# TencentARC/Mix-of-Show

Measured on AMD Instinct MI355X. Metric: edlora_train_images_per_sec_512_sd15, higher is better.
Workload: dtype fp16; 1 GPU; BASELINE.json configs[1]: single-concept ED-LoRA tune, SD-1.5 UNet/CLIP/VAE (random init, calibrated), 512x512, LoRA rank 4 on Attention+CLIPAttention, attn_reg on, batch 4/GPU; global_batch=4, per_gpu_batch=4, image_size=512, parallelism=dp1, grad_bucket_bytes=4466688, preset=sd15, hipgraph=True, channels_last=True

## Files before the change

include/mos_hip.h:

```cpp
#ifndef MOS_HIP_H
#define MOS_HIP_H

#include <stdint.h>

#ifdef __cplusplus
extern "C" {
#endif

typedef enum { MOS_F16 = 0, MOS_BF16 = 1 } mos_dtype;

typedef enum {
    MOS_OK = 0,
    MOS_ERR_BAD_ARG = -1,
    MOS_ERR_UNSUPPORTED = -2,
    MOS_ERR_LAUNCH = -3
} mos_status;

#define MOS_LORA_PAD 16
#define MOS_MAX_PCOLS 4
#define MOS_MAX_SOURCES 9

int mos_version(void);
const char* mos_last_error_string(void);

// ... 75 lines not shown
    mos_lora_grad_out out;
} mos_lora_final_rec;
int mos_lora_linear_fused_bwd_deferred(const void* dy, int64_t lddy, const void* x, int64_t ldx,
                                       const void* Wt, int64_t ldwt, const void* t,
                                       const void* A16T, const void* BpT,
                                       void* dt, void* dx, int64_t lddx,
                                       const mos_lora_grad_out* grads_host, void* ws,
                                       int M, int N, int K, int lora_cols, int dtype, void* stream,
                                       mos_lora_final_rec* rec_host);
int mos_lora_grad_final_all(const mos_lora_final_rec* recs_dev, int n_recs, int total_blocks, void* stream);

typedef struct {
    const void* P[2];
    const void* Z[2];
    int64_t ldz[2];
    int C[2], cb[2];
    float* partial[2];
    int M, rpc, nchunk, nj;
    int block_begin, n_blocks;
    double flops, bytes;
} mos_lora_grad_job;
int mos_lora_linear_fused_bwd_deferred_all(const void* dy, int64_t lddy, const void* x, int64_t ldx,
                                           const void* Wt, int64_t ldwt, const void* t,
                                           const void* A16T, const void* BpT,
                                           void* dt, void* dx, int64_t lddx,
                                           const mos_lora_grad_out* grads_host, void* ws,
                                           int M, int N, int K, int lora_cols, int dtype, void* stream,
                                           mos_lora_final_rec* rec_host, mos_lora_grad_job* job_host);
int mos_lora_grad_all(const mos_lora_grad_job* jobs_dev, int n_jobs, int total_blocks, int nj, int dtype, double flops, double bytes,
                      void* stream);

typedef struct {
    int B, H, Nq, Nkv, d;
    int64_t q_bs, q_rs;
    int64_t k_bs, k_rs;
    int64_t v_bs, v_rs;
    int64_t o_bs, o_rs;
    float scale;
    int causal;
} mos_attn_shape;

int mos_attn_fwd(const void* q, const void* k, const void* v, void* o, float* lse,
                 const int32_t* tok_idx, int n_pcols, float* pcols,
                 const mos_attn_shape* shape_host, int dtype, void* stream);

typedef struct {
    int64_t do_bs, do_rs;
    int64_t dq_bs, dq_rs;
    int64_t dk_bs, dk_rs;
    int64_t dv_bs, dv_rs;
} mos_attn_grad_strides;

int64_t mos_attn_bwd_workspace_bytes(const mos_attn_shape* shape_host);
int mos_attn_bwd(const void* q, const void* k, const void* v, const void* o, const float* lse,
                 const void* dO, const int32_t* tok_idx, int n_pcols, const float* pcols,
                 const float* dpcols, void* dq, void* dk, void* dv, void* ws,
                 const mos_attn_shape* shape_host, const mos_attn_grad_strides* gs_host,
                 int dtype, void* stream);

int mos_self_attn_fwd(const void* q, const void* k, const void* v, void* o, float* lse,
                      const mos_attn_shape* shape_host, int dtype, void* stream);
int mos_cross_attn_fwd(const void* q, const void* k, const void* v, void* o, float* lse,
                       const int32_t* tok_idx, int n_pcols, float* pcols,
                       const mos_attn_shape* shape_host, int dtype, void* stream);
int mos_self_attn_bwd(const void* q, const void* k, const void* v, const void* o, const float* lse, const void* dO,
                      void* dq, void* dk, void* dv, void* ws, const mos_attn_shape* shape_host,
                      const mos_attn_grad_strides* gs_host, int dtype, void* stream);
int mos_cross_attn_bwd(const void* q, const void* k, const void* v, const void* o, const float* lse, const void* dO,
                       const int32_t* tok_idx, int n_pcols, const float* pcols, const float* dpcols,
                       void* dq, void* dk, void* dv, void* ws, const mos_attn_shape* shape_host,
                       const mos_attn_grad_strides* gs_host, int dtype, void* stream);

typedef struct {
    int n_regions;
    int feat_h, feat_w;
    int box[MOS_MAX_SOURCES - 1][4];
    int64_t src_stride;
} mos_region_desc;

int mos_region_cross_attn_fwd(const void* q, const void* k_src, const void* v_src, void* o,
                              const mos_attn_shape* shape_host, const mos_region_desc* reg_host,
                              int dtype, void* stream);
int mos_region_cross_attn_fwd_chunk(const void* q, const void* k_src, const void* v_src, void* o,
                                    const mos_attn_shape* shape_host, const mos_region_desc* reg_host,
                                    const void* total_count, int accumulate, int dtype, void* stream);

int mos_attn_probs(const void* q, const void* k, void* probs, const mos_attn_shape* shape_host, int dtype, void* stream);
int mos_attn_pv(const void* probs, const void* v, void* o, const mos_attn_shape* shape_host, int dtype, void* stream);
int64_t mos_attn_probs_bwd_workspace_bytes(const mos_attn_shape* shape_host);
int mos_attn_pv_bwd(const void* probs, const void* v, const void* dO, void* dprobs, void* dv, void* ws,
                    const mos_attn_shape* shape_host, const mos_attn_grad_strides* gs_host, int dtype, void* stream);
int mos_attn_probs_bwd(const void* q, const void* k, const void* probs, const void* dprobs, void* dq, void* dk, void* ws,
                       const mos_attn_shape* shape_host, const mos_attn_grad_strides* gs_host, int dtype, void* stream);

int64_t mos_gram_workspace_bytes(int64_t n, int Cin, int Cout);
int mos_gram_accumulate(const void* X, int64_t ldx, const void* Y, int64_t ldy, int64_t n,
                        int Cin, int Cout, int dtype, double* G, double* P, double* c,
                        void* ws, void* stream);
int64_t mos_lsq_workspace_bytes(int Cout, int Cin);

int mos_lsq_loss_grad_gram(const double* W, const double* G, const double* P, const double* c,
                           double n_times_cout, int Cout, int Cin, double* loss, double* grad,
                           void* ws, void* stream);

int64_t mos_groupnorm_workspace_bytes(int B, int C, int HW, int G);
int mos_groupnorm_silu_fwd(const void* x, const float* gamma, const float* beta, void* y, float* stats,
// ... 59 lines not shown
```

mix-of-show_amd/csrc/mos_attn.hip:

```cpp
#include <cstdio>
#include <cstdlib>
#include <type_traits>
#include "mos_common.h"

#ifndef MOS_DQ_OCC
#define MOS_DQ_OCC 2
#endif
#ifndef MOS_ATTN_PV16
#define MOS_ATTN_PV16 1
#endif

namespace {

constexpr float LOG2E = 1.4426950408889634f;
constexpr float NEG_BIG = -1.0e30f;
constexpr int KV_TILE = 64;
constexpr int TS = KV_TILE + 8;
__device__ __forceinline__ constexpr int tr_col(int c) { return (c & ~12) | ((c & 4) << 1) | ((c & 8) >> 1); }

__device__ __forceinline__ constexpr int tr_col16(int c) {
    return (c & 32) | ((((c >> 2) & 1) * 2 + ((c >> 4) & 1)) << 3) | (((c >> 3) & 1) << 2) | (c & 3);
}

template <int D>
// ... 1337 lines not shown
        asm volatile("" : "+v"(dvT[0]), "+v"(dkT[0]), "+v"(dvT[1]), "+v"(dkT[1]), "+v"(s1), "+v"(dp1), "+v"(pf1[0]), "+v"(dsf1[0]), "+v"(fdo10[0]), "+v"(fq10[0]), "+v"(fdo10[1]), "+v"(fq10[1]));
        #pragma unroll
        for (int dt = 0; dt < DT; ++dt) { fdo11[dt] = tr_afrag<T>(dOt + (32 * dt + l31) * TS, 1, 1, hh); fq11[dt] = tr_afrag<T>(Qt + (32 * dt + l31) * TS, 1, 1, hh); }
        dvT[0] = MT<T>::mfma32(fdo10[0], pf1[0], dvT[0]);
        { const float p = __builtin_amdgcn_exp2f(s1[8] * c - l1[2][0]); s1[8] = p; dp1[8] = p * dp1[8]; }
        { const float p = __builtin_amdgcn_exp2f(s1[9] * c - l1[2][1]); s1[9] = p; dp1[9] = p * dp1[9]; }
        asm volatile("" : "+v"(dvT[0]), "+v"(dkT[0]), "+v"(dvT[1]), "+v"(dkT[1]), "+v"(s1), "+v"(dp1));
        dkT[0] = MT<T>::mfma32(fq10[0], dsf1[0], dkT[0]);
        { const float p = __builtin_amdgcn_exp2f(s1[10] * c - l1[2][2]); s1[10] = p; dp1[10] = p * dp1[10]; }
        { const float p = __builtin_amdgcn_exp2f(s1[11] * c - l1[2][3]); s1[11] = p; dp1[11] = p * dp1[11]; }
        asm volatile("" : "+v"(dvT[0]), "+v"(dkT[0]), "+v"(dvT[1]), "+v"(dkT[1]), "+v"(s1), "+v"(dp1));
        dvT[1] = MT<T>::mfma32(fdo10[1], pf1[0], dvT[1]);
        { const float p = __builtin_amdgcn_exp2f(s1[12] * c - l1[3][0]); s1[12] = p; dp1[12] = p * dp1[12]; }
        { const float p = __builtin_amdgcn_exp2f(s1[13] * c - l1[3][1]); s1[13] = p; dp1[13] = p * dp1[13]; }
        asm volatile("" : "+v"(dvT[0]), "+v"(dkT[0]), "+v"(dvT[1]), "+v"(dkT[1]), "+v"(s1), "+v"(dp1));
        dkT[1] = MT<T>::mfma32(fq10[1], dsf1[0], dkT[1]);
        { const float p = __builtin_amdgcn_exp2f(s1[14] * c - l1[3][2]); s1[14] = p; dp1[14] = p * dp1[14]; }
        { const float p = __builtin_amdgcn_exp2f(s1[15] * c - l1[3][3]); s1[15] = p; dp1[15] = p * dp1[15]; }
        pf1[1] = acc_to_bfrag<T>(s1, 1); dsf1[1] = acc_to_bfrag<T>(dp1, 1);
        asm volatile("" : "+v"(dvT[0]), "+v"(dkT[0]), "+v"(dvT[1]), "+v"(dkT[1]), "+v"(s1), "+v"(dp1), "+v"(pf1[1]), "+v"(dsf1[1]), "+v"(fdo11[0]), "+v"(fq11[0]), "+v"(fdo11[1]), "+v"(fq11[1]));
        dvT[0] = MT<T>::mfma32(fdo11[0], pf1[1], dvT[0]);
        dkT[0] = MT<T>::mfma32(fq11[0], dsf1[1], dkT[0]);
        dvT[1] = MT<T>::mfma32(fdo11[1], pf1[1], dvT[1]);
        dkT[1] = MT<T>::mfma32(fq11[1], dsf1[1], dkT[1]);
        if (more) store_tile(cur ^ 1);
        __syncthreads();
        cur ^= 1;
    }
    if (a.nsplit == 1) {
        T* dkp = (T*)a.dk + (int64_t)b * a.dk_bs + (int64_t)kvi * a.dk_rs + h * D;
        T* dvp = (T*)a.dv + (int64_t)b * a.dv_bs + (int64_t)kvi * a.dv_rs + h * D;
        store_out_rows<T, D>(dkp, kvalid, dkT, a.scale, hh);
        store_out_rows<T, D>(dvp, kvalid, dvT, 1.0f, hh);
    } else if (kvalid) {
        const int64_t bh = (int64_t)b * a.H + h;
        const int64_t slab = (int64_t)a.B * a.H * a.Nkv * D;
        float* pk = a.part + ((int64_t)split * slab) + (bh * a.Nkv + kvi) * D;
        float* pv = pk + (int64_t)a.nsplit * slab;
#pragma unroll
        for (int dt = 0; dt < DT; ++dt)
#pragma unroll
            for (int r4 = 0; r4 < 4; ++r4) {
                const int db = 32 * dt + 8 * r4 + 4 * hh;
                if (db < D) {
                    *reinterpret_cast<f32x4*>(pk + db) = f32x4{dkT[dt][4 * r4] * a.scale, dkT[dt][4 * r4 + 1] * a.scale,
                                                              dkT[dt][4 * r4 + 2] * a.scale, dkT[dt][4 * r4 + 3] * a.scale};
                    *reinterpret_cast<f32x4*>(pv + db) = f32x4{dvT[dt][4 * r4], dvT[dt][4 * r4 + 1], dvT[dt][4 * r4 + 2],
                                                              dvT[dt][4 * r4 + 3]};
                }
            }
    }
}

template <int D> constexpr int fwd_qw() { return D <= 80 ? 64 : 32; }

template <int D> constexpr size_t fwd_lds(size_t es) { return 2 * (HD<D>::ROW_TILE_ELEMS + HD<D>::TR_TILE_ELEMS) * es; }
template <int D> constexpr size_t dq_lds(size_t es) { return 2 * (2 * HD<D>::ROW_TILE_ELEMS + HD<D>::TR_TILE_ELEMS) * es; }
template <int D> constexpr size_t dkdv_lds(size_t es) {
    return DKDV_NBUF<D>::value * ((2 * HD<D>::ROW_TILE_ELEMS + 2 * HD<D>::TR_TILE_ELEMS) * es +
                                  KV_TILE * (2 + MOS_MAX_PCOLS) * sizeof(float));
}

template <typename K>
void set_lds(K kernel, size_t bytes) {
    if (bytes > 48 * 1024)
        (void)hipFuncSetAttribute(reinterpret_cast<const void*>(kernel), hipFuncAttributeMaxDynamicSharedMemorySize, (int)bytes);
}

int check_shape(const mos_attn_shape* s, const char* who) {
    if (!s) return mos_set_error(MOS_ERR_BAD_ARG, "%s: NULL shape", who);
    if (s->B <= 0 || s->H <= 0 || s->Nq <= 0 || s->Nkv <= 0)
        return mos_set_error(MOS_ERR_BAD_ARG, "%s: B=%d H=%d Nq=%d Nkv=%d", who, s->B, s->H, s->Nq, s->Nkv);
    if (s->d != 40 && s->d != 64 && s->d != 80 && s->d != 160)
        return mos_set_error(MOS_ERR_UNSUPPORTED, "%s: head dim %d not in {40, 64, 80, 160}", who, s->d);
    if (s->causal && s->Nq != s->Nkv)
        return mos_set_error(MOS_ERR_BAD_ARG, "%s: causal masking needs Nq == Nkv (got %d, %d)", who, s->Nq, s->Nkv);
    if (s->q_rs % 8 || s->k_rs % 8 || s->v_rs % 8 || s->o_rs % 4 || s->q_bs % 8 || s->k_bs % 8 || s->v_bs % 8 || s->o_bs % 4)
        return mos_set_error(MOS_ERR_BAD_ARG, "%s: strides must be multiples of 8 elements", who);
    return MOS_OK;
}

AttnArgs make_args(const void* q, const void* k, const void* v, void* o, float* lse, const int32_t* tok, int np,
                   float* pcols, const mos_attn_shape* s, int q_tile) {
    AttnArgs a;
    a.q = q; a.k = k; a.v = v; a.o = o; a.lse = lse; a.tok_idx = tok; a.pcols = pcols; a.n_pcols = np;
    a.B = s->B; a.H = s->H; a.Nq = s->Nq; a.Nkv = s->Nkv; a.nqb = (s->Nq + q_tile - 1) / q_tile;
    a.q_bs = s->q_bs; a.q_rs = s->q_rs; a.k_bs = s->k_bs; a.k_rs = s->k_rs;
    a.v_bs = s->v_bs; a.v_rs = s->v_rs; a.o_bs = s->o_bs; a.o_rs = s->o_rs; a.scale = s->scale;
    a.causal = s->causal;
    return a;
}

template <typename T>
const char* tname() { return sizeof(T) == 2 && std::is_same<T, f16_t>::value ? "f16" : "bf16"; }

struct AttnKey {
    char s[96];
    double flops, bytes;
    AttnKey(const char* dt, const mos_attn_shape* sh, double gemms) {
        snprintf(s, sizeof(s), "%s d%d B%d H%d Nq%d Nkv%d", dt, sh->d, sh->B, sh->H, sh->Nq, sh->Nkv);
        flops = gemms * 2.0 * sh->B * sh->H * (double)sh->Nq * sh->Nkv * sh->d;
        bytes = 2.0 * sh->B * sh->H * sh->d * (2.0 * sh->Nq + 2.0 * sh->Nkv);
    }
};

template <int D> constexpr bool has_causal() { return true; }

template <typename T, int D, int QW, bool PCOLS, bool CAUSAL>
void launch_fwd_one(const AttnArgs& a, size_t lds, hipStream_t st) {
    const dim3 grid((unsigned)(a.H * a.nqb * a.B));
    set_lds(&attn_fwd_kernel<T, D, QW, PCOLS, CAUSAL>, lds);
    hipLaunchKernelGGL((attn_fwd_kernel<T, D, QW, PCOLS, CAUSAL>), grid, dim3(256), lds, st, a);
}
template <typename T, int D, int QW>
void launch_fwd_qw(const AttnArgs& a, int np, size_t lds, hipStream_t st) {
    if constexpr (has_causal<D>()) {
        if (a.causal) {
            if (np > 0) launch_fwd_one<T, D, QW, true, true>(a, lds, st);
            else launch_fwd_one<T, D, QW, false, true>(a, lds, st);
            return;
        }
    }
    if (np > 0) launch_fwd_one<T, D, QW, true, false>(a, lds, st);
    else launch_fwd_one<T, D, QW, false, false>(a, lds, st);
}

template <typename T, int D>
int launch_fwd(const void* q, const void* k, const void* v, void* o, float* lse, const int32_t* tok, int np,
               float* pcols, const mos_attn_shape* s, hipStream_t st) {
    constexpr int QW = fwd_qw<D>();
    const size_t lds = fwd_lds<D>(sizeof(T));
    AttnKey key(tname<T>(), s, 2.0);
    MosProfScope prof(st, np > 0 ? "attn_fwd_pcols" : "attn_fwd", key.s, key.flops, key.bytes);
    const int64_t wg_big = (int64_t)s->H * s->B * ((s->Nq + 4 * QW - 1) / (4 * QW));
    if (QW == 64 && wg_big < 512) {
        launch_fwd_qw<T, D, 32>(make_args(q, k, v, o, lse, tok, np, pcols, s, 128), np, lds, st);
    } else {
        launch_fwd_qw<T, D, QW>(make_args(q, k, v, o, lse, tok, np, pcols, s, 4 * QW), np, lds, st);
    }
    return mos_check_launch("attn_fwd");
}

template <typename T, int D>
int launch_region(const void* q, const void* k, const void* v, void* o, const mos_attn_shape* s,
                  const mos_region_desc* reg, const unsigned char* total_count, int accumulate, hipStream_t st) {
    AttnArgs a = make_args(q, k, v, o, nullptr, nullptr, 0, nullptr, s, 128);
    a.nqb = ((reg->feat_w + 15) / 16) * ((reg->feat_h + 7) / 8);
    const dim3 grid((unsigned)(a.H * a.nqb * a.B));
    const size_t lds = RG<D>::lds_bytes(sizeof(T));
    set_lds(&region_attn_kernel<T, D>, lds);
    double cover = 0.0, area = 0.0;
    for (int r = 0; r < reg->n_regions; ++r) {
        const double bh = reg->box[r][2] - reg->box[r][0], bw = reg->box[r][3] - reg->box[r][1];
        if (bh > 0 && bw > 0) area += bh * bw;
    }
    cover = area + (double)s->Nq;
    AttnKey key(tname<T>(), s, 2.0);
    char rk[128];
    snprintf(rk, sizeof(rk), "%s R%d", key.s, reg->n_regions);
    MosProfScope prof(st, "region_attn", rk, key.flops * cover / (double)s->Nq, key.bytes);
    hipLaunchKernelGGL((region_attn_kernel<T, D>), grid, dim3(256), lds, st, a, *reg, total_count, accumulate);
    return mos_check_launch("region_attn");
}

struct BwdPlan { int nw_q, nw_k, nqb, nkb, nsplit, q_per_split; };
BwdPlan plan_bwd(const mos_attn_shape* s) {
    BwdPlan p;
    p.nw_q = 4;
    p.nw_k = 4;
    p.nqb = (s->Nq + 32 * p.nw_q - 1) / (32 * p.nw_q);
    p.nkb = (s->Nkv + 32 * p.nw_k - 1) / (32 * p.nw_k);
    const int64_t base = (int64_t)p.nkb * s->B * s->H;
    const int qtiles = (s->Nq + KV_TILE - 1) / KV_TILE;
    int ns = (int)((512 + base - 1) / base);
    if (ns > qtiles) ns = qtiles;
    if (ns < 1) ns = 1;
    int tps = (qtiles + ns - 1) / ns;
    ns = (qtiles + tps - 1) / tps;
    p.nsplit = ns;
    p.q_per_split = tps * KV_TILE;
    return p;
}

template <typename T, int D>
int launch_bwd(const void* q, const void* k, const void* v, const void* o, const float* lse, const void* dO,
               const int32_t* tok, int np, const float* pcols, const float* dpcols, void* dq, void* dk, void* dv,
               void* ws, const mos_attn_shape* s, const mos_attn_grad_strides* g, hipStream_t st) {
    const BwdPlan p = plan_bwd(s);
    float* Dvec = (float*)ws;
    const int64_t nrows = (int64_t)s->B * s->H * s->Nq;
    float* part = Dvec + ((nrows + 3) / 4) * 4;
    AttnBwdArgs a;
    a.q = q; a.k = k; a.v = v; a.dO = dO; a.lse = lse; a.Dvec = Dvec; a.tok_idx = tok; a.dpcols = dpcols;
    a.o = o; a.o_bs = s->o_bs; a.o_rs = s->o_rs; a.pcols = pcols;
    a.n_pcols = (dpcols != nullptr && pcols != nullptr) ? np : 0;
    a.dq = dq; a.dk = dk; a.dv = dv; a.part = part;
    a.B = s->B; a.H = s->H; a.Nq = s->Nq; a.Nkv = s->Nkv; a.nqb = p.nqb; a.nkb = p.nkb;
    a.nsplit = p.nsplit; a.q_per_split = p.q_per_split;
    a.q_bs = s->q_bs; a.q_rs = s->q_rs; a.k_bs = s->k_bs; a.k_rs = s->k_rs; a.v_bs = s->v_bs; a.v_rs = s->v_rs;
    a.do_bs = g->do_bs; a.do_rs = g->do_rs; a.dq_bs = g->dq_bs; a.dq_rs = g->dq_rs;
    a.dk_bs = g->dk_bs; a.dk_rs = g->dk_rs; a.dv_bs = g->dv_bs; a.dv_rs = g->dv_rs; a.scale = s->scale;
    a.causal = s->causal;
    const bool pc = a.n_pcols > 0;
    {
        const dim3 grid((unsigned)(a.H * a.nqb * a.B));
        const size_t lds = dq_lds<D>(sizeof(T));
        AttnKey key(tname<T>(), s, 3.0);
        MosProfScope prof(st, "attn_bwd_dq", key.s, key.flops, key.bytes * 1.5);
        auto go = [&](auto pc_c, auto ca_c) {
            constexpr bool PC = decltype(pc_c)::value, CA = decltype(ca_c)::value;
            set_lds(&attn_bwd_dq_kernel<T, D, PC, 4, CA>, lds);
            hipLaunchKernelGGL((attn_bwd_dq_kernel<T, D, PC, 4, CA>), grid, dim3(256), lds, st, a);
        };
        bool done = false;
        if constexpr (has_causal<D>()) {
            if (a.causal) {
                if (pc) go(std::true_type{}, std::true_type{}); else go(std::false_type{}, std::true_type{});
                done = true;
            }
        }
        if (!done) { if (pc) go(std::true_type{}, std::false_type{}); else go(std::false_type{}, std::false_type{}); }
        int rc = mos_check_launch("attn_bwd_dq");
        if (rc) return rc;
    }
    {
        const dim3 grid((unsigned)(a.H * a.nkb * a.B), (unsigned)a.nsplit);
        const size_t lds = dkdv_lds<D>(sizeof(T));
        AttnKey key(tname<T>(), s, 4.0);
        MosProfScope prof(st, "attn_bwd_dkdv", key.s, key.flops, key.bytes * 1.5);
        auto go = [&](auto pc_c, auto ca_c) {
            constexpr bool PC = decltype(pc_c)::value, CA = decltype(ca_c)::value;
            set_lds(&attn_bwd_dkdv_kernel<T, D, PC, 4, CA>, lds);
            hipLaunchKernelGGL((attn_bwd_dkdv_kernel<T, D, PC, 4, CA>), grid, dim3(256), lds, st, a);
        };
        bool done = false;
        if constexpr (D == 40) {
            if (!pc && !a.causal && s->Nq % KV_TILE == 0 && a.q_per_split % KV_TILE == 0) {
                set_lds(&attn_bwd_dkdv_pipe_kernel<T, D>, lds);
                hipLaunchKernelGGL((attn_bwd_dkdv_pipe_kernel<T, D>), grid, dim3(256), lds, st, a);
                done = true;
            }
        }
        if constexpr (has_causal<D>()) {
            if (!done && a.causal) {
                if (pc) go(std::true_type{}, std::true_type{}); else go(std::false_type{}, std::true_type{});
                done = true;
            }
        }
        if (!done) { if (pc) go(std::true_type{}, std::false_type{}); else go(std::false_type{}, std::false_type{}); }
        int rc = mos_check_launch("attn_bwd_dkdv");
        if (rc) return rc;
    }
    if (a.nsplit > 1) {
        const int64_t slab4 = (int64_t)s->B * s->H * s->Nkv * D / 4;
        hipLaunchKernelGGL((attn_bwd_reduce_kernel<T, D>), dim3((unsigned)((slab4 + 255) / 256)), dim3(256), 0, st, part,
                           a.nsplit, (T*)dk, g->dk_bs, g->dk_rs, (T*)dv, g->dv_bs, g->dv_rs, s->B, s->H, s->Nkv);
        return mos_check_launch("attn_bwd_reduce");
    }
    return MOS_OK;
}

#define MOS_DISPATCH_TD(dtype, d, CALL)                                                     \
    do {                                                                                    \
        if ((dtype) == MOS_F16) {                                                           \
            typedef f16_t TT;                                                               \
            if ((d) == 40) { constexpr int DD = 40; return CALL; }                          \
            if ((d) == 64) { constexpr int DD = 64; return CALL; }                          \
            if ((d) == 80) { constexpr int DD = 80; return CALL; }                          \
            if ((d) == 160) { constexpr int DD = 160; return CALL; }                        \
        } else if ((dtype) == MOS_BF16) {                                                   \
            typedef bf16_t TT;                                                              \
            if ((d) == 40) { constexpr int DD = 40; return CALL; }                          \
            if ((d) == 64) { constexpr int DD = 64; return CALL; }                          \
            if ((d) == 80) { constexpr int DD = 80; return CALL; }                          \
            if ((d) == 160) { constexpr int DD = 160; return CALL; }                        \
        }                                                                                   \
        return mos_set_error(MOS_ERR_UNSUPPORTED, "unsupported dtype %d / head dim %d", (int)(dtype), (int)(d)); \
    } while (0)

}

extern "C" {

int mos_attn_fwd(const void* q, const void* k, const void* v, void* o, float* lse, const int32_t* tok_idx, int n_pcols,
                 float* pcols, const mos_attn_shape* s, int dtype, void* stream) {
    int rc = check_shape(s, "mos_attn_fwd");
    if (rc) return rc;
    MOS_REQUIRE(q && k && v && o, "mos_attn_fwd: NULL tensor");
    MOS_REQUIRE(n_pcols >= 0 && n_pcols <= MOS_MAX_PCOLS, "mos_attn_fwd: n_pcols=%d (max %d)", n_pcols, MOS_MAX_PCOLS);
    MOS_REQUIRE(n_pcols == 0 || (tok_idx && pcols), "mos_attn_fwd: n_pcols>0 needs tok_idx and pcols");
    hipStream_t st = (hipStream_t)stream;
    MOS_DISPATCH_TD(dtype, s->d, (launch_fwd<TT, DD>(q, k, v, o, lse, tok_idx, n_pcols, pcols, s, st)));
}

int mos_self_attn_fwd(const void* q, const void* k, const void* v, void* o, float* lse, const mos_attn_shape* s,
                      int dtype, void* stream) {
    return mos_attn_fwd(q, k, v, o, lse, nullptr, 0, nullptr, s, dtype, stream);
}

int mos_cross_attn_fwd(const void* q, const void* k, const void* v, void* o, float* lse, const int32_t* tok_idx,
                       int n_pcols, float* pcols, const mos_attn_shape* s, int dtype, void* stream) {
    return mos_attn_fwd(q, k, v, o, lse, tok_idx, n_pcols, pcols, s, dtype, stream);
}

int64_t mos_attn_bwd_workspace_bytes(const mos_attn_shape* s) {
    if (!s) return 0;
    const BwdPlan p = plan_bwd(s);
    const int64_t nrows = (int64_t)s->B * s->H * s->Nq;
    int64_t fl = ((nrows + 3) / 4) * 4;
    if (p.nsplit > 1) fl += 2 * (int64_t)p.nsplit * s->B * s->H * s->Nkv * s->d;
    return fl * (int64_t)sizeof(float);
}

int mos_attn_bwd(const void* q, const void* k, const void* v, const void* o, const float* lse, const void* dO,
                 const int32_t* tok_idx, int n_pcols, const float* pcols, const float* dpcols, void* dq, void* dk,
                 void* dv, void* ws, const mos_attn_shape* s, const mos_attn_grad_strides* g, int dtype, void* stream) {
    int rc = check_shape(s, "mos_attn_bwd");
    if (rc) return rc;
    MOS_REQUIRE(q && k && v && o && lse && dO && dq && dk && dv && ws && g, "mos_attn_bwd: NULL argument");
    MOS_REQUIRE(n_pcols >= 0 && n_pcols <= MOS_MAX_PCOLS, "mos_attn_bwd: n_pcols=%d", n_pcols);
    MOS_REQUIRE(dpcols == nullptr || (n_pcols > 0 && tok_idx && pcols), "mos_attn_bwd: dpcols needs tok_idx, pcols");
    MOS_REQUIRE(g->do_rs % 8 == 0 && g->dq_rs % 4 == 0 && g->dk_rs % 4 == 0 && g->dv_rs % 4 == 0,
                "mos_attn_bwd: gradient strides misaligned");
    hipStream_t st = (hipStream_t)stream;
    MOS_DISPATCH_TD(dtype, s->d,
                    (launch_bwd<TT, DD>(q, k, v, o, lse, dO, tok_idx, n_pcols, pcols, dpcols, dq, dk, dv, ws, s, g, st)));
}

int mos_self_attn_bwd(const void* q, const void* k, const void* v, const void* o, const float* lse, const void* dO, void* dq,
                      void* dk, void* dv, void* ws, const mos_attn_shape* s, const mos_attn_grad_strides* g, int dtype,
                      void* stream) {
    return mos_attn_bwd(q, k, v, o, lse, dO, nullptr, 0, nullptr, nullptr, dq, dk, dv, ws, s, g, dtype, stream);
}

int mos_cross_attn_bwd(const void* q, const void* k, const void* v, const void* o, const float* lse, const void* dO,
                       const int32_t* tok_idx, int n_pcols, const float* pcols, const float* dpcols, void* dq, void* dk,
                       void* dv, void* ws, const mos_attn_shape* s, const mos_attn_grad_strides* g, int dtype, void* stream) {
    return mos_attn_bwd(q, k, v, o, lse, dO, tok_idx, n_pcols, pcols, dpcols, dq, dk, dv, ws, s, g, dtype, stream);
}

int mos_region_cross_attn_fwd(const void* q, const void* k_src, const void* v_src, void* o, const mos_attn_shape* s,
                              const mos_region_desc* reg, int dtype, void* stream) {
    return mos_region_cross_attn_fwd_chunk(q, k_src, v_src, o, s, reg, nullptr, 0, dtype, stream);
}

int mos_region_cross_attn_fwd_chunk(const void* q, const void* k_src, const void* v_src, void* o, const mos_attn_shape* s,
                                    const mos_region_desc* reg, const void* total_count, int accumulate, int dtype,
                                    void* stream) {
    int rc = check_shape(s, "mos_region_cross_attn_fwd");
    MOS_REQUIRE(!accumulate || total_count, "mos_region_cross_attn_fwd_chunk: accumulate needs the total count map");
    if (rc) return rc;
    MOS_REQUIRE(q && k_src && v_src && o && reg, "mos_region_cross_attn_fwd: NULL argument");
    MOS_REQUIRE(reg->n_regions >= 0 && reg->n_regions <= MOS_MAX_SOURCES - 1, "mos_region_cross_attn_fwd: n_regions=%d",
                reg->n_regions);
    MOS_REQUIRE(reg->feat_h > 0 && reg->feat_w > 0 && reg->feat_h * reg->feat_w == s->Nq,
                "mos_region_cross_attn_fwd: feat %dx%d != Nq %d", reg->feat_h, reg->feat_w, s->Nq);
    if (s->Nkv <= 64 || s->Nkv > 96)
// ... 9 lines not shown
```

mix-of-show_amd/mixofshow/hip/lib.py:

```python
import ctypes
import os
import threading

_HERE = os.path.dirname(os.path.abspath(__file__))
LIB_PATH = os.environ.get('MOS_HIP_LIB') or os.path.normpath(os.path.join(_HERE, '..', '..', 'libmos_hip.so'))

MOS_F16 = 0
MOS_BF16 = 1
MOS_LORA_PAD = 16
MOS_MAX_PCOLS = 4
MOS_MAX_SOURCES = 9


class MosHipUnavailable(RuntimeError):
    pass


class MosHipError(RuntimeError):
    pass


class LoraSites(ctypes.Structure):
    _fields_ = [
        ('n_sites', ctypes.c_int),
# ... 63 lines not shown
    ]


class AttnGradStrides(ctypes.Structure):
    _fields_ = [
        ('do_bs', ctypes.c_int64), ('do_rs', ctypes.c_int64),
        ('dq_bs', ctypes.c_int64), ('dq_rs', ctypes.c_int64),
        ('dk_bs', ctypes.c_int64), ('dk_rs', ctypes.c_int64),
        ('dv_bs', ctypes.c_int64), ('dv_rs', ctypes.c_int64),
    ]


class RegionDesc(ctypes.Structure):
    _fields_ = [
        ('n_regions', ctypes.c_int),
        ('feat_h', ctypes.c_int), ('feat_w', ctypes.c_int),
        ('box', (ctypes.c_int * 4) * (MOS_MAX_SOURCES - 1)),
        ('src_stride', ctypes.c_int64),
    ]


_vp, _i, _i64, _f, _d = ctypes.c_void_p, ctypes.c_int, ctypes.c_int64, ctypes.c_float, ctypes.c_double

SIGNATURES = {
    'mos_version': (_i, []),
    'mos_last_error_string': (ctypes.c_char_p, []),
    'mos_profile_begin': (_i, []),
    'mos_profile_end': (_i, []),
    'mos_profile_get': (_i, [_i, ctypes.c_char_p, _i, ctypes.POINTER(ctypes.c_double),
                             ctypes.POINTER(ctypes.c_longlong), ctypes.POINTER(ctypes.c_double),
                             ctypes.POINTER(ctypes.c_double)]),
    'mos_lora_pack': (_i, [ctypes.POINTER(LoraSites), _i, _vp, _vp, _vp, _vp, _vp]),
    'mos_lora_pack_all': (_i, [_vp, _i, _i, _i, _vp]),
    'mos_lora_linear_fused_fwd': (_i, [_vp, _i64, _vp, _i64, _vp, _vp, _vp, _vp, _i64, _vp, _i, _i, _i, _i, _vp]),
    'mos_lora_linear_fwd_ex': (_i, [_vp, _i64, _vp, _i64, _vp, _vp, _vp, _vp, _i64, _vp, _i, _i, _i, _i,
                                    ctypes.POINTER(GemmEpilogue), _vp]),
    'mos_lora_linear_fused_bwd': (_i, [_vp, _i64, _vp, _i64, _vp, _i64, _vp, _vp, _vp, _vp, _vp, _i64,
                                       ctypes.POINTER(LoraGradOut), _vp, _i, _i, _i, _i, _i, _vp]),
    'mos_lora_linear_fused_bwd_deferred': (_i, [_vp, _i64, _vp, _i64, _vp, _i64, _vp, _vp, _vp, _vp, _vp, _i64,
                                                ctypes.POINTER(LoraGradOut), _vp, _i, _i, _i, _i, _i, _vp,
                                                ctypes.POINTER(LoraFinalRec)]),
    'mos_lora_linear_fused_bwd_deferred_all': (_i, [_vp, _i64, _vp, _i64, _vp, _i64, _vp, _vp, _vp, _vp, _vp, _i64,
                                                ctypes.POINTER(LoraGradOut), _vp, _i, _i, _i, _i, _i, _vp,
                                                ctypes.POINTER(LoraFinalRec), ctypes.POINTER(LoraGradJob)]),
    'mos_lora_grad_all': (_i, [_vp, _i, _i, _i, _i, ctypes.c_double, ctypes.c_double, _vp]),
    'mos_lora_grad_final_all': (_i, [_vp, _i, _i, _vp]),
    'mos_lora_down': (_i, [_vp, _i64, _vp, _vp, _i, _i, _i, _vp]),
    'mos_lora_linear_fwd': (_i, [_vp, _i64, _vp, _i64, _vp, _vp, _vp, _vp, _i64, _i, _i, _i, _i, _vp]),
    'mos_lora_bwd_workspace_bytes': (_i64, [_i, _i, _i]),
    'mos_lora_linear_bwd': (_i, [_vp, _i64, _vp, _i64, _vp, _i64, _vp, _vp, _vp, _vp, _vp, _i64, _vp, _vp, _vp,
                                 _i, _i, _i, _i, _i, _vp]),
    'mos_attn_fwd': (_i, [_vp, _vp, _vp, _vp, _vp, _vp, _i, _vp, ctypes.POINTER(AttnShape), _i, _vp]),
    'mos_attn_bwd_workspace_bytes': (_i64, [ctypes.POINTER(AttnShape)]),
    'mos_attn_bwd': (_i, [_vp, _vp, _vp, _vp, _vp, _vp, _vp, _i, _vp, _vp, _vp, _vp, _vp, _vp,
                          ctypes.POINTER(AttnShape), ctypes.POINTER(AttnGradStrides), _i, _vp]),
    'mos_self_attn_fwd': (_i, [_vp, _vp, _vp, _vp, _vp, ctypes.POINTER(AttnShape), _i, _vp]),
    'mos_cross_attn_fwd': (_i, [_vp, _vp, _vp, _vp, _vp, _vp, _i, _vp, ctypes.POINTER(AttnShape), _i, _vp]),
    'mos_region_cross_attn_fwd': (_i, [_vp, _vp, _vp, _vp, ctypes.POINTER(AttnShape), ctypes.POINTER(RegionDesc),
                                       _i, _vp]),
    'mos_region_cross_attn_fwd_chunk': (_i, [_vp, _vp, _vp, _vp, ctypes.POINTER(AttnShape), ctypes.POINTER(RegionDesc),
                                             _vp, _i, _i, _vp]),
    'mos_attn_probs': (_i, [_vp, _vp, _vp, ctypes.POINTER(AttnShape), _i, _vp]),
    'mos_attn_pv': (_i, [_vp, _vp, _vp, ctypes.POINTER(AttnShape), _i, _vp]),
    'mos_attn_probs_bwd_workspace_bytes': (_i64, [ctypes.POINTER(AttnShape)]),
    'mos_attn_pv_bwd': (_i, [_vp, _vp, _vp, _vp, _vp, _vp, ctypes.POINTER(AttnShape), ctypes.POINTER(AttnGradStrides), _i, _vp]),
    'mos_attn_probs_bwd': (_i, [_vp, _vp, _vp, _vp, _vp, _vp, _vp, ctypes.POINTER(AttnShape), ctypes.POINTER(AttnGradStrides),
                                _i, _vp]),
    'mos_self_attn_bwd': (_i, [_vp, _vp, _vp, _vp, _vp, _vp, _vp, _vp, _vp, _vp, ctypes.POINTER(AttnShape),
                               ctypes.POINTER(AttnGradStrides), _i, _vp]),
    'mos_cross_attn_bwd': (_i, [_vp, _vp, _vp, _vp, _vp, _vp, _vp, _i, _vp, _vp, _vp, _vp, _vp, _vp, ctypes.POINTER(AttnShape),
                                ctypes.POINTER(AttnGradStrides), _i, _vp]),
    'mos_gram_workspace_bytes': (_i64, [_i64, _i, _i]),
    'mos_gram_accumulate': (_i, [_vp, _i64, _vp, _i64, _i64, _i, _i, _i, _vp, _vp, _vp, _vp, _vp]),
    'mos_groupnorm_workspace_bytes': (_i64, [_i, _i, _i, _i]),
    'mos_groupnorm_silu_fwd': (_i, [_vp, _vp, _vp, _vp, _vp, _vp, _i, _i, _i, _i, _f, _i, _i, _vp]),
    'mos_groupnorm_silu_bwd': (_i, [_vp, _vp, _vp, _vp, _vp, _vp, _vp, _i, _i, _i, _i, _i, _i, _vp]),
    'mos_groupnorm_nhwc_workspace_bytes': (_i64, [_i, _i, _i, _i]),
    'mos_groupnorm_silu_fwd_nhwc': (_i, [_vp, _vp, _vp, _vp, _vp, _vp, _i, _i, _i, _i, _f, _i, _i, _vp]),
    'mos_groupnorm_silu_bwd_nhwc': (_i, [_vp, _vp, _vp, _vp, _vp, _vp, _vp, _i, _i, _i, _i, _i, _i, _vp]),
    'mos_groupnorm_silu_bwd_nhwc_res_ps': (_i, [_vp, _vp, _i64, _vp, _vp, _vp, _vp, _vp, _vp, _i, _i, _i, _i, _i, _i, _vp]),
    'mos_groupnorm_silu_bwd_nhwc_res': (_i, [_vp, _vp, _vp, _vp, _vp, _vp, _vp, _vp, _i, _i, _i, _i, _i, _i, _vp]),
    'mos_conv3x3_nhwc': (_i, [_vp, _vp, _vp, _vp, _vp, _vp, _i, _i, _i, _i, _i, _i, _i, _vp]),
    'mos_conv3x3_nhwc_workspace_bytes': (_i64, [_i, _i, _i, _i, _i]),
    'mos_conv3x3_gn_tiles': (_i, [_i, _i, _i, _i, _i]),
    'mos_conv3x3_nhwc_px': (_i, [_vp, _i64, _vp, _vp, _vp, _vp, _vp, _i, _i, _i, _i, _i, _i, _i, _vp, _vp, _vp]),
    'mos_conv3x3_nhwc_gn': (_i, [_vp, _vp, _vp, _vp, _vp, _vp, _i, _i, _i, _i, _i, _i, _i, _vp, _vp, _vp]),
    'mos_groupnorm_nhwc_reads_twice': (_i, [_i, _i, _i, _i]),
    'mos_groupnorm_silu_fwd_nhwc_pre': (_i, [_vp, _vp, _i, _vp, _vp, _vp, _vp, _vp, _i, _i, _i, _i, _f, _i, _i, _vp]),
    'mos_conv3x3_s2_nhwc': (_i, [_vp, _vp, _vp, _vp, _i, _i, _i, _i, _i, _i, _i, _vp, _vp]),
    'mos_conv3x3_nhwc_ws': (_i, [_vp, _vp, _vp, _vp, _vp, _vp, _i, _i, _i, _i, _i, _i, _i, _vp, _vp]),
    'mos_layernorm_fwd': (_i, [_vp, _vp, _vp, _vp, _vp, _i, _i, _f, _i, _vp]),
    'mos_layernorm_bwd': (_i, [_vp, _vp, _vp, _vp, _vp, _i, _i, _i, _vp]),
    'mos_add_layernorm_fwd': (_i, [_vp, _vp, _vp, _vp, _vp, _vp, _vp, _i, _i, _f, _i, _i, _vp]),
    'mos_add_layernorm_bwd': (_i, [_vp, _vp, _vp, _vp, _vp, _vp, _vp, _i, _i, _i, _i, _vp]),
    'mos_geglu_fwd': (_i, [_vp, _vp, _i64, _i, _i, _vp]),
    'mos_softmax_rows': (_i, [_vp, _vp, _i, _i, _f, _i, _vp]),
    'mos_geglu_bwd': (_i, [_vp, _vp, _vp, _i64, _i, _i, _vp]),
    'mos_quick_gelu_fwd': (_i, [_vp, _vp, _i64, _i, _vp]),
    'mos_quick_gelu_bwd': (_i, [_vp, _vp, _vp, _i64, _i, _vp]),
    'mos_lsq_workspace_bytes': (_i64, [_i, _i]),
    'mos_lsq_loss_grad_gram': (_i, [_vp, _vp, _vp, _vp, _d, _i, _i, _vp, _vp, _vp, _vp]),
}

_lib = None
_lock = threading.Lock()

# ... 29 lines not shown
```

Before: 127.0 images/s.

## Add single-block attention kernels for short sequences up to 80 tokens

Adds dedicated forward and backward attention kernels for head dim 64 and sequence lengths up to 80, with one workgroup per (batch, head). K/V are staged once in LDS and the full softmax is computed without online rescaling. The backward computes dq, dk and dv in one kernel, with no workspace or split reduction. This targets CLIP text-encoder attention, where the general tiled path wastes launches and tile padding. The risks are added code paths and LDS-heavy workgroups with limited occupancy.

```diff
diff --git a/include/mos_hip.h b/include/mos_hip.h
--- a/include/mos_hip.h
+++ b/include/mos_hip.h
@@ -151,6 +151,7 @@
 } mos_attn_grad_strides;
 
 int64_t mos_attn_bwd_workspace_bytes(const mos_attn_shape* shape_host);
+int mos_attn_short_form(const mos_attn_shape* shape_host, int n_pcols);
 int mos_attn_bwd(const void* q, const void* k, const void* v, const void* o, const float* lse,
                  const void* dO, const int32_t* tok_idx, int n_pcols, const float* pcols,
                  const float* dpcols, void* dq, void* dk, void* dv, void* ws,
diff --git a/mix-of-show_amd/csrc/mos_attn.hip b/mix-of-show_amd/csrc/mos_attn.hip
--- a/mix-of-show_amd/csrc/mos_attn.hip
+++ b/mix-of-show_amd/csrc/mos_attn.hip
@@ -1413,6 +1413,8 @@
     }
 }
 
+#include "mos_attn_short.inc"
+
 template <int D> constexpr int fwd_qw() { return D <= 80 ? 64 : 32; }
 
 template <int D> constexpr size_t fwd_lds(size_t es) { return 2 * (HD<D>::ROW_TILE_ELEMS + HD<D>::TR_TILE_ELEMS) * es; }
@@ -1486,9 +1488,34 @@
     else launch_fwd_one<T, D, QW, false, false>(a, lds, st);
 }
 
+bool short_form(const mos_attn_shape* s, int np) {
+#ifdef MOS_ATTN_NO_SHORT
+    return false;
+#endif
+    if (!s || np != 0 || s->d != SH_D) return false;
+    if (s->Nq < 1 || s->Nq > SH_N || s->Nkv < 1 || s->Nkv > SH_N) return false;
+    if (s->causal && s->Nq != s->Nkv) return false;
+    return s->q_rs <= SH_MAX_STRIDE && s->k_rs <= SH_MAX_STRIDE && s->v_rs <= SH_MAX_STRIDE && s->o_rs <= SH_MAX_STRIDE &&
+           s->q_rs >= 0 && s->k_rs >= 0 && s->v_rs >= 0 && s->o_rs >= 0;
+}
+
+template <typename T>
+int launch_short_fwd(const void* q, const void* k, const void* v, void* o, float* lse, const mos_attn_shape* s, hipStream_t st) {
+    const AttnArgs a = make_args(q, k, v, o, lse, nullptr, 0, nullptr, s, SH_N);
+    const size_t lds = short_fwd_lds(sizeof(T));
+    AttnKey key(tname<T>(), s, 2.0);
+    MosProfScope prof(st, "attn_fwd", key.s, key.flops, key.bytes);
+    set_lds(&attn_short_fwd_kernel<T>, lds);
+    hipLaunchKernelGGL((attn_short_fwd_kernel<T>), dim3((unsigned)(s->B * s->H)), dim3(SH_NT), lds, st, a);
+    return mos_check_launch("attn_short_fwd");
+}
+
 template <typename T, int D>
 int launch_fwd(const void* q, const void* k, const void* v, void* o, float* lse, const int32_t* tok, int np,
                float* pcols, const mos_attn_shape* s, hipStream_t st) {
+    if constexpr (D == SH_D) {
+        if (short_form(s, np)) return launch_short_fwd<T>(q, k, v, o, lse, s, st);
+    }
     constexpr int QW = fwd_qw<D>();
     const size_t lds = fwd_lds<D>(sizeof(T));
     AttnKey key(tname<T>(), s, 2.0);
@@ -1562,6 +1589,16 @@
     a.do_bs = g->do_bs; a.do_rs = g->do_rs; a.dq_bs = g->dq_bs; a.dq_rs = g->dq_rs;
     a.dk_bs = g->dk_bs; a.dk_rs = g->dk_rs; a.dv_bs = g->dv_bs; a.dv_rs = g->dv_rs; a.scale = s->scale;
     a.causal = s->causal;
+    if constexpr (D == SH_D) {
+        if (short_form(s, np) && g->do_rs >= 0 && g->do_rs <= SH_MAX_STRIDE) {
+            const size_t lds = short_bwd_lds(sizeof(T));
+            AttnKey key(tname<T>(), s, 5.0);
+            MosProfScope prof(st, "attn_bwd_short", key.s, key.flops, key.bytes * 2.0);
+            set_lds(&attn_short_bwd_kernel<T>, lds);
+            hipLaunchKernelGGL((attn_short_bwd_kernel<T>), dim3((unsigned)(s->B * s->H)), dim3(SH_NT), lds, st, a);
+            return mos_check_launch("attn_short_bwd");
+        }
+    }
     const bool pc = a.n_pcols > 0;
     {
         const dim3 grid((unsigned)(a.H * a.nqb * a.B));
@@ -1664,6 +1701,8 @@
     return mos_attn_fwd(q, k, v, o, lse, tok_idx, n_pcols, pcols, s, dtype, stream);
 }
 
+int mos_attn_short_form(const mos_attn_shape* s, int n_pcols) { return short_form(s, n_pcols) ? 1 : 0; }
+
 int64_t mos_attn_bwd_workspace_bytes(const mos_attn_shape* s) {
     if (!s) return 0;
     const BwdPlan p = plan_bwd(s);
diff --git a/mix-of-show_amd/csrc/mos_attn_short.inc b/mix-of-show_amd/csrc/mos_attn_short.inc
--- /dev/null
+++ b/mix-of-show_amd/csrc/mos_attn_short.inc
@@ -0,0 +1,259 @@
+
+constexpr int SH_N = 80;
+constexpr int SH_D = 64;
+constexpr int SH_NT = 320;
+constexpr int SH_RS = SH_D + 8;
+constexpr int SH_TS = SH_N + 8;
+constexpr int SH_ROW = SH_N * SH_RS;
+constexpr int SH_TR = SH_D * SH_TS;
+constexpr int SH_PT = SH_N * SH_TS;
+constexpr int64_t SH_MAX_STRIDE = 1 << 20;
+
+constexpr size_t short_fwd_lds(size_t es) { return (size_t)(SH_ROW + SH_TR) * es; }
+constexpr size_t short_bwd_lds(size_t es) {
+    return (size_t)((2 * SH_ROW + SH_TR) > (2 * SH_TR + 2 * SH_PT) ? (2 * SH_ROW + SH_TR) : (2 * SH_TR + 2 * SH_PT)) * es;
+}
+
+struct ShortPair { u32x4 r0, r1; };
+template <typename T>
+__device__ __forceinline__ ShortPair short_load_pair(rsrc_t src, int rs, int tid) {
+    const int p = tid % 40, cc = tid / 40;
+    const int off = (2 * p * rs + cc * 8) * (int)sizeof(T);
+    ShortPair s;
+    s.r0 = ldbuf16(src, off);
+    s.r1 = ldbuf16(src, off + rs * (int)sizeof(T));
+    return s;
+}
+template <typename T>
+__device__ __forceinline__ void short_store_rows(T* lds, const ShortPair& s, int tid) {
+    const int p = tid % 40, cc = tid / 40;
+    st16(lds + (2 * p) * SH_RS + cc * 8, s.r0);
+    st16(lds + (2 * p + 1) * SH_RS + cc * 8, s.r1);
+}
+template <typename T>
+__device__ __forceinline__ void short_store_tr(T* ldsT, const ShortPair& s, int tid) {
+    const int p = tid % 40, cc = tid / 40;
+    uint32_t* dst = reinterpret_cast<uint32_t*>(ldsT + (cc * 8) * SH_TS + 2 * p);
+#pragma unroll
+    for (int w = 0; w < 4; ++w) {
+        dst[(2 * w) * (SH_TS / 2)] = __builtin_amdgcn_perm(s.r1[w], s.r0[w], 0x05040100u);
+        dst[(2 * w + 1) * (SH_TS / 2)] = __builtin_amdgcn_perm(s.r1[w], s.r0[w], 0x07060302u);
+    }
+}
+template <typename T>
+__device__ __forceinline__ typename MT<T>::v4 short_ld4(const T* p) { return __builtin_bit_cast(typename MT<T>::v4, ld8(p)); }
+
+template <typename T>
+__global__ __launch_bounds__(SH_NT, 3) void attn_short_fwd_kernel(AttnArgs a) {
+    typedef typename MT<T>::v8 v8;
+    typedef typename MT<T>::v4 v4;
+    extern __shared__ __attribute__((aligned(16))) unsigned char smem_raw[];
+    T* Ks = reinterpret_cast<T*>(smem_raw);
+    T* Vt = Ks + SH_ROW;
+    const int tid = threadIdx.x, lane = tid & 63, w = tid >> 6, li = lane & 15, g = lane >> 4;
+    const int h = blockIdx.x % a.H, b = blockIdx.x / a.H;
+    const int qi = 16 * w + li;
+    const rsrc_t qsrc = make_rsrc((const T*)a.q + (int64_t)b * a.q_bs + h * SH_D, slice_bytes<T, SH_D>(a.Nq, a.q_rs));
+    const rsrc_t ksrc = make_rsrc((const T*)a.k + (int64_t)b * a.k_bs + h * SH_D, slice_bytes<T, SH_D>(a.Nkv, a.k_rs));
+    const rsrc_t vsrc = make_rsrc((const T*)a.v + (int64_t)b * a.v_bs + h * SH_D, slice_bytes<T, SH_D>(a.Nkv, a.v_rs));
+    const ShortPair kp = short_load_pair<T>(ksrc, (int)a.k_rs, tid);
+    const ShortPair vp = short_load_pair<T>(vsrc, (int)a.v_rs, tid);
+    v8 qf[2];
+#pragma unroll
+    for (int ks = 0; ks < 2; ++ks) qf[ks] = as_v8<T>(ldbuf16(qsrc, (qi * (int)a.q_rs + 32 * ks + 8 * g) * (int)sizeof(T)));
+    short_store_rows<T>(Ks, kp, tid);
+    short_store_tr<T>(Vt, vp, tid);
+    __syncthreads();
+    if (16 * w >= a.Nq) return;
+    const int nkt = (a.Nkv + 15) >> 4;
+    const int tlast = a.causal ? min(w, nkt - 1) : nkt - 1;
+    const int klim = a.causal ? min(qi, a.Nkv - 1) : a.Nkv - 1;
+    const float c = a.scale * LOG2E;
+    f32x4 s[5];
+    float mx = NEG_BIG;
+#pragma unroll
+    for (int t = 0; t < 5; ++t) {
+        s[t] = f32x4{NEG_BIG, NEG_BIG, NEG_BIG, NEG_BIG};
+        if (t <= tlast) {
+            const T* krow = Ks + (16 * t + li) * SH_RS + 8 * g;
+            const v8 a0 = as_v8<T>(ld16(krow)), a1 = as_v8<T>(ld16(krow + 32));
+            f32x4 acc = MT<T>::mfma16(a0, qf[0], f32x4{0.f, 0.f, 0.f, 0.f});
+            acc = MT<T>::mfma16(a1, qf[1], acc);
+#pragma unroll
+            for (int r = 0; r < 4; ++r) {
+                s[t][r] = (16 * t + 4 * g + r > klim) ? NEG_BIG : acc[r];
+                mx = fmaxf(mx, s[t][r]);
+            }
+        }
+    }
+    mx = fmaxf(mx, __shfl_xor(mx, 16));
+    mx = fmaxf(mx, __shfl_xor(mx, 32));
+    const float mc = mx * c;
+    float ls = 0.f;
+    f32x4 o[4];
+#pragma unroll
+    for (int dm = 0; dm < 4; ++dm) o[dm] = f32x4{0.f, 0.f, 0.f, 0.f};
+#pragma unroll
+    for (int t = 0; t < 5; ++t) {
+        if (t <= tlast) {
+            float p[4];
+#pragma unroll
+            for (int r = 0; r < 4; ++r) {
+                p[r] = __builtin_amdgcn_exp2f(s[t][r] * c - mc);
+                ls += p[r];
+            }
+            const v4 pf = __builtin_bit_cast(v4, pack4<T>(p[0], p[1], p[2], p[3]));
+#pragma unroll
+            for (int dm = 0; dm < 4; ++dm)
+                o[dm] = MT<T>::mfma16k16(short_ld4<T>(Vt + (16 * dm + li) * SH_TS + 16 * t + 4 * g), pf, o[dm]);
+        }
+    }
+    ls += __shfl_xor(ls, 16);
+    ls += __shfl_xor(ls, 32);
+    if (qi < a.Nq) {
+        const float inv = 1.0f / ls;
+        T* orow = (T*)a.o + (int64_t)b * a.o_bs + (int64_t)qi * a.o_rs + h * SH_D;
+#pragma unroll
+        for (int dm = 0; dm < 4; ++dm)
+            st8(orow + 16 * dm + 4 * g, pack4<T>(o[dm][0] * inv, o[dm][1] * inv, o[dm][2] * inv, o[dm][3] * inv));
+        if (a.lse != nullptr && g == 0) a.lse[((int64_t)b * a.H + h) * a.Nq + qi] = mx * a.scale + __logf(ls);
+    }
+}
+
+template <typename T>
+__global__ __launch_bounds__(SH_NT, 3) void attn_short_bwd_kernel(AttnBwdArgs a) {
+    typedef typename MT<T>::v8 v8;
+    typedef typename MT<T>::v4 v4;
+    extern __shared__ __attribute__((aligned(16))) unsigned char smem_raw[];
+    T* Ks = reinterpret_cast<T*>(smem_raw);
+    T* Vs = Ks + SH_ROW;
+    T* Kt = Vs + SH_ROW;
+    T* Qt = reinterpret_cast<T*>(smem_raw);
+    T* dOt = Qt + SH_TR;
+    T* Pt = dOt + SH_TR;
+    T* dSt = Pt + SH_PT;
+    const int tid = threadIdx.x, lane = tid & 63, w = tid >> 6, li = lane & 15, g = lane >> 4;
+    const int h = blockIdx.x % a.H, b = blockIdx.x / a.H;
+    const int qi = 16 * w + li;
+    const bool qvalid = qi < a.Nq;
+    const rsrc_t qsrc = make_rsrc((const T*)a.q + (int64_t)b * a.q_bs + h * SH_D, slice_bytes<T, SH_D>(a.Nq, a.q_rs));
+    const rsrc_t dosrc = make_rsrc((const T*)a.dO + (int64_t)b * a.do_bs + h * SH_D, slice_bytes<T, SH_D>(a.Nq, a.do_rs));
+    const rsrc_t osrc = make_rsrc((const T*)a.o + (int64_t)b * a.o_bs + h * SH_D, slice_bytes<T, SH_D>(a.Nq, a.o_rs));
+    const rsrc_t ksrc = make_rsrc((const T*)a.k + (int64_t)b * a.k_bs + h * SH_D, slice_bytes<T, SH_D>(a.Nkv, a.k_rs));
+    const rsrc_t vsrc = make_rsrc((const T*)a.v + (int64_t)b * a.v_bs + h * SH_D, slice_bytes<T, SH_D>(a.Nkv, a.v_rs));
+    const ShortPair kp = short_load_pair<T>(ksrc, (int)a.k_rs, tid);
+    const ShortPair vp = short_load_pair<T>(vsrc, (int)a.v_rs, tid);
+    v8 qf[2], dof[2], of[2];
+#pragma unroll
+    for (int ks = 0; ks < 2; ++ks) {
+        const int col = 32 * ks + 8 * g;
+        qf[ks] = as_v8<T>(ldbuf16(qsrc, (qi * (int)a.q_rs + col) * (int)sizeof(T)));
+        dof[ks] = as_v8<T>(ldbuf16(dosrc, (qi * (int)a.do_rs + col) * (int)sizeof(T)));
+        of[ks] = as_v8<T>(ldbuf16(osrc, (qi * (int)a.o_rs + col) * (int)sizeof(T)));
+    }
+    const float lse2 = a.lse[((int64_t)b * a.H + h) * a.Nq + min(qi, a.Nq - 1)] * LOG2E;
+    short_store_rows<T>(Ks, kp, tid);
+    short_store_tr<T>(Kt, kp, tid);
+    short_store_rows<T>(Vs, vp, tid);
+    float Dq = 0.f;
+#pragma unroll
+    for (int ks = 0; ks < 2; ++ks)
+#pragma unroll
+        for (int e = 0; e < 8; ++e) Dq += (float)of[ks][e] * (float)dof[ks][e];
+    Dq += __shfl_xor(Dq, 16);
+    Dq += __shfl_xor(Dq, 32);
+    __syncthreads();
+
+    const int nkt = (a.Nkv + 15) >> 4, nqt = (a.Nq + 15) >> 4;
+    const float c = a.scale * LOG2E;
+    u32x2 pk[5], dsk[5];
+#pragma unroll
+    for (int t = 0; t < 5; ++t) { pk[t] = u32x2{0u, 0u}; dsk[t] = u32x2{0u, 0u}; }
+    if (w < nqt) {
+        const int tlast = a.causal ? min(w, nkt - 1) : nkt - 1;
+        const int klim = a.causal ? min(qi, a.Nkv - 1) : a.Nkv - 1;
+        f32x4 dq[4];
+#pragma unroll
+        for (int dm = 0; dm < 4; ++dm) dq[dm] = f32x4{0.f, 0.f, 0.f, 0.f};
+#pragma unroll
+        for (int t = 0; t < 5; ++t) {
+            if (t <= tlast) {
+                const T* krow = Ks + (16 * t + li) * SH_RS + 8 * g;
+                const T* vrow = Vs + (16 * t + li) * SH_RS + 8 * g;
+                const v8 ak0 = as_v8<T>(ld16(krow)), ak1 = as_v8<T>(ld16(krow + 32));
+                const v8 av0 = as_v8<T>(ld16(vrow)), av1 = as_v8<T>(ld16(vrow + 32));
+                f32x4 s = MT<T>::mfma16(ak0, qf[0], f32x4{0.f, 0.f, 0.f, 0.f});
+                f32x4 dp = MT<T>::mfma16(av0, dof[0], f32x4{-Dq, -Dq, -Dq, -Dq});
+                s = MT<T>::mfma16(ak1, qf[1], s);
+                dp = MT<T>::mfma16(av1, dof[1], dp);
+                float p[4], ds[4];
+#pragma unroll
+                for (int r = 0; r < 4; ++r) {
+                    const bool keep = qvalid && (16 * t + 4 * g + r <= klim);
+                    p[r] = keep ? __builtin_amdgcn_exp2f(s[r] * c - lse2) : 0.f;
+                    ds[r] = p[r] * dp[r];
+                }
+                pk[t] = pack4<T>(p[0], p[1], p[2], p[3]);
+                dsk[t] = pack4<T>(ds[0], ds[1], ds[2], ds[3]);
+                const v4 dsf = __builtin_bit_cast(v4, dsk[t]);
+#pragma unroll
+                for (int dm = 0; dm < 4; ++dm)
+                    dq[dm] = MT<T>::mfma16k16(short_ld4<T>(Kt + (16 * dm + li) * SH_TS + 16 * t + 4 * g), dsf, dq[dm]);
+            }
+        }
+        if (qvalid) {
+            T* dqrow = (T*)a.dq + (int64_t)b * a.dq_bs + (int64_t)qi * a.dq_rs + h * SH_D;
+#pragma unroll
+            for (int dm = 0; dm < 4; ++dm)
+                st8(dqrow + 16 * dm + 4 * g, pack4<T>(dq[dm][0] * a.scale, dq[dm][1] * a.scale, dq[dm][2] * a.scale,
+                                                       dq[dm][3] * a.scale));
+        }
+    }
+    __syncthreads();
+#pragma unroll
+    for (int ks = 0; ks < 2; ++ks)
+#pragma unroll
+        for (int e = 0; e < 8; ++e) {
+            Qt[(32 * ks + 8 * g + e) * SH_TS + qi] = qf[ks][e];
+            dOt[(32 * ks + 8 * g + e) * SH_TS + qi] = dof[ks][e];
+        }
+#pragma unroll
+    for (int t = 0; t < 5; ++t) {
+        const T* ph = reinterpret_cast<const T*>(&pk[t]);
+        const T* dh = reinterpret_cast<const T*>(&dsk[t]);
+#pragma unroll
+        for (int r = 0; r < 4; ++r) {
+            Pt[(16 * t + 4 * g + r) * SH_TS + qi] = ph[r];
+            dSt[(16 * t + 4 * g + r) * SH_TS + qi] = dh[r];
+        }
+    }
+    __syncthreads();
+    if (w >= nkt) return;
+    const int kvi = 16 * w + li;
+    const int t0 = a.causal ? w : 0;
+    f32x4 dk[4], dv[4];
+#pragma unroll
+    for (int dm = 0; dm < 4; ++dm) { dk[dm] = f32x4{0.f, 0.f, 0.f, 0.f}; dv[dm] = f32x4{0.f, 0.f, 0.f, 0.f}; }
+#pragma unroll
+    for (int tq = 0; tq < 5; ++tq) {
+        if (tq >= t0 && tq < nqt) {
+            const v4 pB = short_ld4<T>(Pt + kvi * SH_TS + 16 * tq + 4 * g);
+            const v4 dsB = short_ld4<T>(dSt + kvi * SH_TS + 16 * tq + 4 * g);
+#pragma unroll
+            for (int dm = 0; dm < 4; ++dm) {
+                dv[dm] = MT<T>::mfma16k16(short_ld4<T>(dOt + (16 * dm + li) * SH_TS + 16 * tq + 4 * g), pB, dv[dm]);
+                dk[dm] = MT<T>::mfma16k16(short_ld4<T>(Qt + (16 * dm + li) * SH_TS + 16 * tq + 4 * g), dsB, dk[dm]);
+            }
+        }
+    }
+    if (kvi < a.Nkv) {
+        T* dkrow = (T*)a.dk + (int64_t)b * a.dk_bs + (int64_t)kvi * a.dk_rs + h * SH_D;
+        T* dvrow = (T*)a.dv + (int64_t)b * a.dv_bs + (int64_t)kvi * a.dv_rs + h * SH_D;
+#pragma unroll
+        for (int dm = 0; dm < 4; ++dm) {
+            st8(dkrow + 16 * dm + 4 * g, pack4<T>(dk[dm][0] * a.scale, dk[dm][1] * a.scale, dk[dm][2] * a.scale,
+                                                   dk[dm][3] * a.scale));
+            st8(dvrow + 16 * dm + 4 * g, pack4<T>(dv[dm][0], dv[dm][1], dv[dm][2], dv[dm][3]));
+        }
+    }
+}
diff --git a/mix-of-show_amd/mixofshow/hip/lib.py b/mix-of-show_amd/mixofshow/hip/lib.py
--- a/mix-of-show_amd/mixofshow/hip/lib.py
+++ b/mix-of-show_amd/mixofshow/hip/lib.py
@@ -139,6 +139,7 @@
                                  _i, _i, _i, _i, _i, _vp]),
     'mos_attn_fwd': (_i, [_vp, _vp, _vp, _vp, _vp, _vp, _i, _vp, ctypes.POINTER(AttnShape), _i, _vp]),
     'mos_attn_bwd_workspace_bytes': (_i64, [ctypes.POINTER(AttnShape)]),
+    'mos_attn_short_form': (_i, [ctypes.POINTER(AttnShape), _i]),
     'mos_attn_bwd': (_i, [_vp, _vp, _vp, _vp, _vp, _vp, _vp, _i, _vp, _vp, _vp, _vp, _vp, _vp,
                           ctypes.POINTER(AttnShape), ctypes.POINTER(AttnGradStrides), _i, _vp]),
     'mos_self_attn_fwd': (_i, [_vp, _vp, _vp, _vp, _vp, ctypes.POINTER(AttnShape), _i, _vp]),
```

Measured after the change: 128.3 images/s (median of 6 runs). 1.1% higher.
